# zhoupengwei/tloam

Measured on AMD Instinct MI355X. Metric: gauss_newton_iters_per_sec, higher is better.
Workload: dtype f64

## Files before the change

### tloam_amd/csrc/tl_walk.hpp

```cpp
#pragma once

#include "tl_common.hpp"
#include "tl_knn.hpp"

#ifndef TL_K1_STAMP
#define TL_K1_STAMP(i)
#endif

namespace tl {

template <int K, int LPQ>
__device__ __forceinline__ void knn_rows(const GridView& g, const PtsGlobal& pts, Vec3 pw, int sub, TopK<K>& tk,
                                         int2* __restrict__ lds_rows, double radius, NbrXyz<K>* xyz = nullptr) {
  TL_K1_STAMP(1)
  const int cx = cell_coord(pw.x, g.org[0], g.inv_cell, g.dim[0]);
  const int cy = cell_coord(pw.y, g.org[1], g.inv_cell, g.dim[1]);
  const int cz = cell_coord(pw.z, g.org[2], g.inv_cell, g.dim[2]);
  int x0 = cx - 1;
  if (x0 < 0) x0 = 0;
  constexpr int NR = (9 + LPQ - 1) / LPQ;
  int rs[NR], re[NR];
  const double cl = g.cell, reach = radius * (1.0 + 1e-6), c2 = reach * reach;
  const double fx = (pw.x - g.org[0]) * g.inv_cell - (double)cx, fy = (pw.y - g.org[1]) * g.inv_cell - (double)cy,
               fz = (pw.z - g.org[2]) * g.inv_cell - (double)cz;
  const double dxl = fx * cl, dxr = (1.0 - fx) * cl, dyl = fy * cl, dyr = (1.0 - fy) * cl, dzl = fz * cl, dzr = (1.0 - fz) * cl;
  const double sxl = dxl * dxl, sxr = dxr * dxr, syl = dyl * dyl, syr = dyr * dyr, szl = dzl * dzl, szr = dzr * dzr;
  typedef int int4u __attribute__((ext_vector_type(4), aligned(4)));
#pragma unroll
  for (int i = 0; i < NR; ++i) {
    const int r = sub + i * LPQ;
    const int rz = r / 3, ry = r % 3;
    const int z = cz - 1 + rz, y = cy - 1 + ry;
    const double s2 = (rz == 0 ? szl : (rz == 2 ? szr : 0.0)) + (ry == 0 ? syl : (ry == 2 ? syr : 0.0));
    int xa = cx - ((s2 + sxl <= c2) ? 1 : 0), xb = cx + ((s2 + sxr <= c2) ? 1 : 0);
    if (xa < 0) xa = 0;
    if (xb >= g.dim[0]) xb = g.dim[0] - 1;
    const bool in = (r < 9) && (s2 <= c2) && (xa <= xb) && z >= 0 && z < g.dim[2] && y >= 0 && y < g.dim[1];
    const size_t base = in ? ((size_t)z * g.dim[1] + y) * g.dim[0] + x0 : 0;
    const int4u t = *reinterpret_cast<const int4u*>(g.cell_start + base);
    const int ia = xa - x0, ib = xb + 1 - x0;
    rs[i] = in ? (ia == 0 ? t.x : t.y) : 0;
    re[i] = in ? (ib == 3 ? t.w : (ib == 2 ? t.z : t.y)) : 0;
  }
  topk_clear<K>(tk);
  TL_K1_STAMP(2)
  if (LPQ == 1) {
    const int lane = threadIdx.x & 63;
    int nr = 0, total = 0;
#pragma unroll
    for (int i = 0; i < NR; ++i) {
      const int len = re[i] - rs[i];
      if (len > 0) {
        lds_rows[nr * 64 + lane] = int2{rs[i], re[i]};
        ++nr;
        total += len;
      }
    }
    int j = 0, e = 0, r = 0;
    int2 nx = (nr > 0) ? lds_rows[lane] : int2{0, 0};
    const unsigned keep_mask = ~((1u << key_bits_for(g.n)) - 1u);
    KeyList<K + 1> L;
    keys_clear<K + 1>(L);
    auto next = [&](int& jx, bool& vx) {
      if (j >= e && r < nr) { j = nx.x; e = nx.y; ++r; nx = lds_rows[(r < nr ? r : 0) * 64 + lane]; }
      vx = j < e;
      jx = vx ? j : 0;
      j += vx ? 1 : 0;
    };
#ifndef TLOAM_K1_CPT
#define TLOAM_K1_CPT 4
#endif
    constexpr int kCpt = TLOAM_K1_CPT;
    int jc[kCpt];
    bool vc[kCpt];
    double4 rc[kCpt];
#pragma unroll
    for (int u = 0; u < kCpt; ++u) next(jc[u], vc[u]);
#pragma unroll
    for (int u = 0; u < kCpt; ++u) rc[u] = pts.p[jc[u]];
#ifdef TLOAM_K1_DBG_NOWALK
    total = 0;
#endif
#ifdef TLOAM_K1_DBG_MAXTRIPS
    int trip_no = 0;
    for (int left = total; __any(left > 0) && trip_no < TLOAM_K1_DBG_MAXTRIPS; left -= kCpt, ++trip_no) {
#else
    for (int left = total; __any(left > 0); left -= kCpt) {
#endif
      int jn[kCpt];
      bool vn[kCpt];
      double4 rn[kCpt];
#pragma unroll
      for (int u = 0; u < kCpt; ++u) next(jn[u], vn[u]);
#pragma unroll
      for (int u = 0; u < kCpt; ++u) rn[u] = pts.p[jn[u]];
#pragma unroll
      for (int u = 0; u < kCpt; ++u) {
        const double du = sqdist(pw.x, pw.y, pw.z, rc[u].x, rc[u].y, rc[u].z);
        key_insert<K + 1>(L, key_pack(du, jc[u], keep_mask, vc[u]));
      }
#pragma unroll
      for (int u = 0; u < kCpt; ++u) { jc[u] = jn[u]; vc[u] = vn[u]; rc[u] = rn[u]; }
    }
    if (!keys_ambiguous<K + 1>(L, keep_mask)) {
      keys_unpack<K, K + 1>(L, pts, pw.x, pw.y, pw.z, keep_mask, tk, xyz);
    } else {
      topk_clear<K>(tk);
      for (int q = 0; q < nr; ++q) {
        const int2 v = lds_rows[q * 64 + lane];
        scan_range<K>(pts, v.x, v.y, pw.x, pw.y, pw.z, tk);
      }
      if (xyz) nbr_fetch<K>(pts, tk, xyz);
    }
  } else {
    const unsigned keep_mask = ~((1u << key_bits_for(g.n)) - 1u);
    KeyList<K + 1> L;
    keys_clear<K + 1>(L);
    int len = 0;
#pragma unroll
    for (int i = 0; i < NR; ++i) len = max(len, re[i] - rs[i]);
#ifndef TLOAM_K1_WIDE_KU
#define TLOAM_K1_WIDE_KU 4
#endif
    constexpr int kU = (NR == 1) ? TLOAM_K1_WIDE_KU : 2;
#ifdef TLOAM_K1_DBG_NOWALK
    len = 0;
#endif
    for (int s = 0; s < len; s += kU) {
      double4 c[kU][NR];
#pragma unroll
      for (int u = 0; u < kU; ++u)
#pragma unroll
        for (int i = 0; i < NR; ++i) c[u][i] = pts.p[(rs[i] + s + u < re[i]) ? rs[i] + s + u : 0];
#pragma unroll
      for (int u = 0; u < kU; ++u)
#pragma unroll
        for (int i = 0; i < NR; ++i) {
          const bool v = rs[i] + s + u < re[i];
          key_insert<K + 1>(L, key_pack(sqdist(pw.x, pw.y, pw.z, c[u][i].x, c[u][i].y, c[u][i].z), rs[i] + s + u, keep_mask, v));
        }
    }
    TL_K1_STAMP(3)
#ifndef TLOAM_K1_DBG_NOMERGE
#pragma unroll
    for (int x = 1; x < LPQ; x <<= 1) {
      double ok[K + 1];
#pragma unroll
      for (int m = 0; m < K + 1; ++m) ok[m] = __shfl_xor(L.k[m], x, 64);
#pragma unroll
      for (int m = 0; m < K + 1; ++m) key_insert<K + 1>(L, ok[m]);
    }
#endif
    TL_K1_STAMP(4)
    if (!keys_ambiguous<K + 1>(L, keep_mask)) {
      keys_unpack<K, K + 1>(L, pts, pw.x, pw.y, pw.z, keep_mask, tk, xyz);
      TL_K1_STAMP(5)
    } else {
      for (int s = 0; s < len; ++s) {
        double4 c[NR];
#pragma unroll
        for (int i = 0; i < NR; ++i) c[i] = pts.p[(rs[i] + s < re[i]) ? rs[i] + s : 0];
#pragma unroll
        for (int i = 0; i < NR; ++i)
          if (rs[i] + s < re[i])
            topk_insert<K, PtsGlobal>(tk, pts, sqdist(pw.x, pw.y, pw.z, c[i].x, c[i].y, c[i].z), rs[i] + s);
      }
#pragma unroll
      for (int x = 1; x < LPQ; x <<= 1) {
        double od[K];
        int oj[K];
#pragma unroll
        for (int m = 0; m < K; ++m) { od[m] = __shfl_xor(tk.d[m], x, 64); oj[m] = __shfl_xor(tk.j[m], x, 64); }
#pragma unroll
        for (int m = 0; m < K; ++m)
          if (oj[m] >= 0) topk_insert<K, PtsGlobal>(tk, pts, od[m], oj[m]);
      }
      if (xyz) nbr_fetch<K>(pts, tk, xyz);
    }
  }
}

}
```

Before: 61650.

## Balance multi-lane KNN walk by flattening candidate rows across lane group

In the multi-lane-per-query path, each lane previously walked its own subset of cell rows up to the longest row, so lanes with short rows idled. The new code gathers all nine row ranges across the lane group with shuffles, builds a prefix-sum mapping from a flat candidate index to a point index, and strides lanes over the combined candidate list. Work is now spread evenly across the group. In exchange, each candidate pays an 8-step index remap, and the unroll factors change to 3.

```diff
diff --git a/tloam_amd/csrc/tl_walk.hpp b/tloam_amd/csrc/tl_walk.hpp
--- a/tloam_amd/csrc/tl_walk.hpp
+++ b/tloam_amd/csrc/tl_walk.hpp
@@ -116,29 +116,46 @@
     const unsigned keep_mask = ~((1u << key_bits_for(g.n)) - 1u);
     KeyList<K + 1> L;
     keys_clear<K + 1>(L);
-    int len = 0;
-#pragma unroll
-    for (int i = 0; i < NR; ++i) len = max(len, re[i] - rs[i]);
+    const int g0 = (int)__lane_id() - sub;
+    int end[8], gap[8];
+    int a0 = 0, total = 0, prev = 0;
+#pragma unroll
+    for (int r = 0; r < 9; ++r) {
+      const int a = __shfl(rs[r / LPQ], g0 + r % LPQ, 64), b = __shfl(re[r / LPQ], g0 + r % LPQ, 64);
+      if (r == 0) a0 = a;
+      else gap[r - 1] = a - prev;
+      total += b - a;
+      prev = b;
+      if (r < 8) end[r] = total;
+    }
+    auto rec_of = [&](int p) {
+      int j = p + a0;
+#pragma unroll
+      for (int r = 0; r < 8; ++r) j += (p >= end[r]) ? gap[r] : 0;
+      return j;
+    };
 #ifndef TLOAM_K1_WIDE_KU
-#define TLOAM_K1_WIDE_KU 4
-#endif
-    constexpr int kU = (NR == 1) ? TLOAM_K1_WIDE_KU : 2;
+#define TLOAM_K1_WIDE_KU 3
+#endif
+#ifndef TLOAM_K1_QUAD_KU
+#define TLOAM_K1_QUAD_KU 3
+#endif
+    constexpr int kU = (LPQ == 16) ? TLOAM_K1_WIDE_KU : TLOAM_K1_QUAD_KU;
 #ifdef TLOAM_K1_DBG_NOWALK
-    len = 0;
-#endif
-    for (int s = 0; s < len; s += kU) {
-      double4 c[kU][NR];
+    total = 0;
+#endif
+    for (int s = sub; s < total; s += LPQ * kU) {
+      int j[kU];
+      double4 c[kU];
+#pragma unroll
+      for (int u = 0; u < kU; ++u) {
+        const int p = s + u * LPQ;
+        j[u] = (p < total) ? rec_of(p) : 0;
+        c[u] = pts.p[j[u]];
+      }
 #pragma unroll
       for (int u = 0; u < kU; ++u)
-#pragma unroll
-        for (int i = 0; i < NR; ++i) c[u][i] = pts.p[(rs[i] + s + u < re[i]) ? rs[i] + s + u : 0];
-#pragma unroll
-      for (int u = 0; u < kU; ++u)
-#pragma unroll
-        for (int i = 0; i < NR; ++i) {
-          const bool v = rs[i] + s + u < re[i];
-          key_insert<K + 1>(L, key_pack(sqdist(pw.x, pw.y, pw.z, c[u][i].x, c[u][i].y, c[u][i].z), rs[i] + s + u, keep_mask, v));
-        }
+        key_insert<K + 1>(L, key_pack(sqdist(pw.x, pw.y, pw.z, c[u].x, c[u].y, c[u].z), j[u], keep_mask, s + u * LPQ < total));
     }
     TL_K1_STAMP(3)
 #ifndef TLOAM_K1_DBG_NOMERGE
@@ -156,6 +173,9 @@
       keys_unpack<K, K + 1>(L, pts, pw.x, pw.y, pw.z, keep_mask, tk, xyz);
       TL_K1_STAMP(5)
     } else {
+      int len = 0;
+#pragma unroll
+      for (int i = 0; i < NR; ++i) len = max(len, re[i] - rs[i]);
       for (int s = 0; s < len; ++s) {
         double4 c[NR];
 #pragma unroll
```

After: 63970, median of 6. +3.8%, better.
